# steineggerlab/unicore

Hardware: AMD Instinct MI355X
Metric: 3Di alignments/sec (cluster path) (higher is better)
Workload: dtype u16

## Files before the change

unicore_amd/csrc/uc_align.hip:

```cpp
#include <mutex>
#include <hip/hip_runtime.h>

#include <cmath>

#include <algorithm>
#include <cstdlib>
#include <cstring>

#include <rocprim/rocprim.hpp>

#include "uc_engine.h"

namespace uc {

constexpr int SW_PK_OVF_HOST = 0x7C00 - 256;

struct TbBudget {
    unsigned long long forced = 0;
    TbBudget() {
        if (const char *e = getenv("UC_TB_BUDGET_MB")) forced = std::max<unsigned long long>(1, strtoull(e, nullptr, 10)) << 20;
    }
    uint32_t segment_pairs() const { return forced ? 1000u : (32u << 20); }
    unsigned long long batch_bytes(unsigned long long total, size_t held) const {
        if (forced) return forced;
        size_t free_b = 0, total_b = 0;
        unsigned long long cap = 64ull << 30;
        if (hipMemGetInfo(&free_b, &total_b) == hipSuccess)
            cap = std::min<unsigned long long>(cap, (unsigned long long)((free_b + held) * 0.55));
        const unsigned long long budget = std::max<unsigned long long>(cap, 256ull << 20);
        if (held >= ((size_t)8 << 30)) return (unsigned long long)held - 64;
        const unsigned long long want = std::max<unsigned long long>(16ull << 30, total / 3);
        return std::min(budget, std::max<unsigned long long>(want, (unsigned long long)held));
    }
};

namespace {

constexpr int MAXCLS = 28;
struct ClassTable {
    int n;
    int cap[MAXCLS], G[MAXCLS], R[MAXCLS], pk[MAXCLS];
    uint32_t tcap[MAXCLS];
};
const ClassTable h_tab[4] = {
    {16,
     {64, 128, 192, 256, 320, 384, 448, 512, 640, 768, 896, 1024, 1280, 1536, 1792, 2048},
     {16, 16, 16, 16, 16, 16, 16, 16, 32, 32, 32, 32, 64, 64, 64, 64},
     {4, 8, 12, 16, 20, 24, 28, 32, 20, 24, 28, 32, 20, 24, 28, 32},
     {0, 0, 0, 0, 0, 0, 0, 0, 0, 0, 0, 0, 0, 0, 0, 0},
     {256, 256, 256, 256, 256, 256, 256, 256, 64, 64, 64, 64, 24, 24, 24, 24}},
    {28,
     {32, 64, 96, 128, 160, 192, 224, 256, 288, 320, 352, 384, 448, 512, 576, 640, 704, 768, 896, 1024, 1152, 1280, 1408, 1536, 1664, 1792, 1920, 2048},
     {16, 16, 16, 16, 16, 16, 16, 16, 16, 16, 16, 16, 32, 32, 32, 32, 32, 32, 64, 64, 64, 64, 64, 64, 64, 64, 64, 64},
     {2, 4, 6, 8, 10, 12, 14, 16, 18, 20, 22, 24, 14, 16, 18, 20, 22, 24, 14, 16, 18, 20, 22, 24, 26, 28, 30, 32},
     {1, 1, 1, 1, 1, 1, 1, 1, 1, 1, 1, 1, 1, 1, 1, 1, 1, 1, 1, 1, 1, 1, 1, 1, 1, 1, 1, 1},
     {64, 64, 64, 64, 64, 64, 64, 64, 64, 64, 64, 64, 64, 64, 64, 64, 64, 64, 48, 48, 48, 48, 48, 48, 24, 24, 24, 24}},
    {12,
     {64, 128, 192, 256, 384, 512, 768, 1024, 1280, 1536, 1792, 2048},
     {16, 16, 16, 16, 32, 32, 64, 64, 64, 64, 64, 64},
     {4, 8, 12, 16, 12, 16, 12, 16, 20, 24, 28, 32},
     {0, 0, 0, 0, 0, 0, 0, 0, 0, 0, 0, 0},
     {256, 256, 256, 256, 64, 64, 24, 24, 24, 24, 24, 24}},
    {16,
     {128, 256, 384, 512, 640, 768, 896, 1024, 1152, 1280, 1408, 1536, 1664, 1792, 1920, 2048},
     {64, 64, 64, 64, 64, 64, 64, 64, 64, 64, 64, 64, 64, 64, 64, 64},
     {2, 4, 6, 8, 10, 12, 14, 16, 18, 20, 22, 24, 26, 28, 30, 32},
     {1, 1, 1, 1, 1, 1, 1, 1, 1, 1, 1, 1, 1, 1, 1, 1},
     {8, 8, 8, 8, 8, 8, 16, 16, 16, 16, 16, 16, 16, 16, 16, 16}},
};
__device__ __constant__ ClassTable c_tab[4];
static int pk_known_tab(uint32_t n_pairs, uint32_t n_queries) {
    static const bool on = !(getenv("UC_SW_SPARSE") && atoi(getenv("UC_SW_SPARSE")) == 0);
    return on && (double)n_pairs < 2.5 * (double)n_queries ? 3 : 1;
}

__device__ __forceinline__ int class_of(int lq, int tab) {
    int c = 0;
    while (c < c_tab[tab].n && c_tab[tab].cap[c] < lq) c++;
    return c;
}
__device__ __forceinline__ uint32_t task_cap(int c, int tab) { return c < c_tab[tab].n ? c_tab[tab].tcap[c] : SW_LONG_TASK_PAIRS; }

__global__ void __launch_bounds__(256) plan_key_kernel(uint32_t n, const uint32_t *q, const uint32_t *t, const int32_t *qe,
                                                       const int32_t *te, const int32_t *qs, const int32_t *ts,
                                                       const uint32_t *len, int tab, uint64_t *key, uint32_t *idx,
                                                       unsigned long long *alg_bytes ) {
    unsigned long long bytes = 0, cells = 0;
    for (uint32_t i = blockIdx.x * 256 + threadIdx.x; i < n; i += gridDim.x * 256) {
        const uint32_t qq = q[i];
        const uint32_t lq = len[qq];
        const uint32_t tl = te ? (uint32_t)(te[i] + 1 - (ts ? ts[i] : 0)) : len[t[i]];
        const uint32_t ql = qe ? (uint32_t)(qe[i] + 1 - (qs ? qs[i] : 0)) : lq;
        key[i] = ((uint64_t)class_of((int)lq, tab) << 40) | ((uint64_t)qq << 16) | (uint64_t)(65535u - tl);
        idx[i] = i;
        bytes += 2ull * (ql + tl) + 32;
        cells += (unsigned long long)ql * tl;
    }
    for (int o = 32; o > 0; o >>= 1) { bytes += __shfl_down(bytes, o, 64); cells += __shfl_down(cells, o, 64); }
    if ((threadIdx.x & 63) == 0 && bytes) { atomicAdd(alg_bytes, bytes); atomicAdd(alg_bytes + 1, cells); }
}

__global__ void __launch_bounds__(256) plan_gather_kernel(uint32_t n, const uint64_t *key, const uint32_t *idx, const uint32_t *t,
                                                          const int32_t *qe, const int32_t *te, const int32_t *qs, const int32_t *ts,
                                                          uint32_t *sq, uint32_t *st, int32_t *sqe, int32_t *ste, int32_t *sqs,
                                                          int32_t *sts, uint32_t *head) {
    for (uint32_t i = blockIdx.x * 256 + threadIdx.x; i < n; i += gridDim.x * 256) {
        const uint64_t k = key[i];
        const uint32_t o = idx[i];
        sq[i] = (uint32_t)(k >> 16) & 0xFFFFFFu;
        st[i] = t[o];
        if (qe) { sqe[i] = qe[o]; ste[i] = te[o]; }
        if (qs) { sqs[i] = qs[o]; sts[i] = ts[o]; }
        head[i] = (i == 0 || (key[i - 1] >> 16) != (k >> 16)) ? i : 0u;
    }
}

__global__ void __launch_bounds__(256) plan_aux_kernel(uint32_t n, const uint32_t *idx, const int32_t *aux, int32_t *saux) {
    for (uint32_t i = blockIdx.x * 256 + threadIdx.x; i < n; i += gridDim.x * 256) saux[i] = aux[idx[i]];
}

__global__ void __launch_bounds__(256) plan_taskflag_kernel(uint32_t n, const uint64_t *key, const uint32_t *segstart, int tab, uint32_t *flag) {
    for (uint32_t i = blockIdx.x * 256 + threadIdx.x; i < n; i += gridDim.x * 256)
        flag[i] = ((i - segstart[i]) % task_cap((int)(key[i] >> 40), tab)) == 0 ? 1u : 0u;
}

__global__ void __launch_bounds__(256) plan_taskfill_kernel(uint32_t n, const uint64_t *key, const uint32_t *flag, const uint32_t *tpos,
                                                            SwTask *tasks, uint32_t *tcls) {
    for (uint32_t i = blockIdx.x * 256 + threadIdx.x; i < n; i += gridDim.x * 256) {
        if (!flag[i]) continue;
        const uint64_t k = key[i];
        const uint32_t w = tpos[i];
        tasks[w].q = (uint32_t)(k >> 16) & 0xFFFFFFu;
        tasks[w].begin = i;
        tcls[w] = (uint32_t)(k >> 40);
    }
}

__global__ void __launch_bounds__(256) plan_taskcount_kernel(uint32_t ntasks, uint32_t n, SwTask *tasks, const uint32_t *tcls,
                                                             const uint64_t *key, uint64_t *tkey, uint32_t *tidx) {
    for (uint32_t k = blockIdx.x * 256 + threadIdx.x; k < ntasks; k += gridDim.x * 256) {
        const uint32_t b = tasks[k].begin;
        const uint32_t cnt = (k + 1 < ntasks ? tasks[k + 1].begin : n) - b;
        tasks[k].count = cnt;
        const uint32_t work = cnt * (65535u - (uint32_t)(key[b] & 0xFFFF));
        tkey[k] = ((uint64_t)tcls[k] << 32) | (uint64_t)(0xFFFFFFFFu - work);
        tidx[k] = k;
    }
}

__global__ void __launch_bounds__(256) plan_taskgather_kernel(uint32_t ntasks, const uint32_t *tidx, const SwTask *in, SwTask *out) {
    for (uint32_t k = blockIdx.x * 256 + threadIdx.x; k < ntasks; k += gridDim.x * 256) out[k] = in[tidx[k]];
}

constexpr int NB = MAXCLS + 2;
__global__ void plan_bounds_kernel(uint32_t ntasks, const uint32_t *tcls, uint32_t n, const uint64_t *key, uint32_t *bounds) {
    const uint32_t c = threadIdx.x;
// ... 581 lines not shown
    UC_HIP(hipStreamSynchronize(E.stream));
    return a + b;
}

struct PackedPrefix { uint32_t pairs, tasks; };
static PackedPrefix packed_prefix(const SwPlan &P) {
    const ClassTable &tab = h_tab[P.tab];
    int c = 0;
    while (c < tab.n && tab.pk[c]) c++;
    return {P.pair_base[c], P.task_base[c]};
}

static void build_plan(Engine &E, SwPlan &P, DevBuf<char> &tmp, uint32_t n, const uint32_t *q, const uint32_t *t,
                       const int32_t *qe, const int32_t *te, int tab, const int32_t *qs = nullptr, const int32_t *ts = nullptr,
                       const int32_t *aux = nullptr ,
                       bool lpt = true ) {
    {
        static std::mutex mu;
        static bool uploaded[64] = {};
        std::lock_guard<std::mutex> g(mu);
        if (E.device < 0 || E.device >= 64 || !uploaded[E.device]) {
            ClassTable t[4];
            memcpy(t, h_tab, sizeof t);
            UC_HIP(hipMemcpyToSymbol(HIP_SYMBOL(c_tab), t, sizeof t));
            if (E.device >= 0 && E.device < 64) uploaded[E.device] = true;
        }
    }
    P.n = n; P.ntasks = 0; P.alg_bytes = 0; P.cells = 0; P.has_ends = qe != nullptr; P.has_starts = qs != nullptr; P.tab = tab;
    P.has_aux = aux != nullptr;
    memset(P.task_base, 0, sizeof P.task_base);
    memset(P.pair_base, 0, sizeof P.pair_base);
    if (!n) return;
    hipStream_t s = E.stream;
    P.key.reserve(n); P.key2.reserve(n); P.idx_in.reserve(n); P.idx.reserve(n);
    P.sq.reserve(n); P.st.reserve(n); P.head.reserve(n); P.segstart.reserve(n); P.flag.reserve(n); P.tpos.reserve(n);
    if (qe) { P.sqe.reserve(n); P.ste.reserve(n); }
    if (qs) { P.sqs.reserve(n); P.sts.reserve(n); }
    P.bytes.reserve(2); P.bounds.reserve(2 * NB);
    UC_HIP(hipMemsetAsync(P.bytes.p, 0, 16, s));
    hipLaunchKernelGGL(plan_key_kernel, grid_for(n), dim3(256), 0, s, n, q, t, qe, te, qs, ts, E.ddb.len, tab, P.key.p, P.idx_in.p, P.bytes.p);
    rocprim_call(tmp, [&](void *t, size_t &b) { return rocprim::radix_sort_pairs(t, b, P.key.p, P.key2.p, P.idx_in.p, P.idx.p, (size_t)n, 0u, 45u, s); });
    hipLaunchKernelGGL(plan_gather_kernel, grid_for(n), dim3(256), 0, s, n, P.key2.p, P.idx.p, t, qe, te, qs, ts, P.sq.p, P.st.p, P.sqe.p, P.ste.p, P.sqs.p, P.sts.p, P.head.p);
    if (aux) {
        P.saux.reserve(n);
        hipLaunchKernelGGL(plan_aux_kernel, grid_for(n), dim3(256), 0, s, n, P.idx.p, aux, P.saux.p);
    }
    max_scan_u32(E, tmp, P.head.p, P.segstart.p, n);
    hipLaunchKernelGGL(plan_taskflag_kernel, grid_for(n), dim3(256), 0, s, n, P.key2.p, P.segstart.p, tab, P.flag.p);
    P.ntasks = compact(E, tmp, P.flag.p, P.tpos.p, n);
    P.tasks.reserve(P.ntasks); P.tcls.reserve(P.ntasks);
    hipLaunchKernelGGL(plan_taskfill_kernel, grid_for(n), dim3(256), 0, s, n, P.key2.p, P.flag.p, P.tpos.p, P.tasks.p, P.tcls.p);
    P.tasks_in.reserve(P.ntasks); P.tkey.reserve(P.ntasks); P.tkey2.reserve(P.ntasks); P.tidx.reserve(P.ntasks); P.tidx2.reserve(P.ntasks);
    hipLaunchKernelGGL(plan_taskcount_kernel, grid_for(P.ntasks), dim3(256), 0, s, P.ntasks, n, P.tasks.p, P.tcls.p, P.key2.p, P.tkey.p, P.tidx.p);
    if (lpt) {
        rocprim_call(tmp, [&](void *t, size_t &b) { return rocprim::radix_sort_pairs(t, b, P.tkey.p, P.tkey2.p, P.tidx.p, P.tidx2.p, (size_t)P.ntasks, 0u, 37u, s); });
        UC_HIP(hipMemcpyAsync(P.tasks_in.p, P.tasks.p, (size_t)P.ntasks * sizeof(SwTask), hipMemcpyDeviceToDevice, s));
        hipLaunchKernelGGL(plan_taskgather_kernel, grid_for(P.ntasks), dim3(256), 0, s, P.ntasks, P.tidx2.p, P.tasks_in.p, P.tasks.p);
    }
    hipLaunchKernelGGL(plan_bounds_kernel, dim3(1), dim3(64), 0, s, P.ntasks, P.tcls.p, n, P.key2.p, P.bounds.p);
    uint32_t hb[2 * NB];
    unsigned long long bytes[2] = {0, 0};
    UC_HIP(hipMemcpyAsync(hb, P.bounds.p, sizeof hb, hipMemcpyDeviceToHost, s));
    UC_HIP(hipMemcpyAsync(bytes, P.bytes.p, 16, hipMemcpyDeviceToHost, s));
    UC_HIP(hipStreamSynchronize(s));
    UC_HIP(hipGetLastError());
    memcpy(P.task_base, hb, NB * 4);
    memcpy(P.pair_base, hb + NB, NB * 4);
    P.alg_bytes = bytes[0];
    P.cells = bytes[1];
}

static uint64_t launch_plan(Engine &E, SwPlan &P, int mode, int32_t *os, int32_t *oqe, int32_t *ote, DevBuf<int32_t> &work,
                            const uint32_t *tb = nullptr, bool only_long = false, uint32_t t0 = 0, uint32_t t1 = 0xFFFFFFFFu, bool skip_long = false) {
    const ClassTable &tab = h_tab[P.tab];
    SwArgs a;
    a.db = E.ddb; a.tasks = P.tasks.p; a.pt = P.st.p; a.pqe = P.sqe.p; a.pte = P.ste.p;
    a.pqs = P.has_starts ? P.sqs.p : nullptr; a.pts = P.has_starts ? P.sts.p : nullptr;
    a.oscore = os; a.oqe = oqe; a.ote = ote; a.open = E.p.gap_open; a.ext = E.p.gap_ext;
    if (tb) { a.tb_diag = tb[0]; a.tb_ident = tb[1]; a.tb_open = tb[2]; a.tb_ext = tb[3]; }
    a.pscore = P.has_aux ? P.saux.p : nullptr;
    const int imode = mode >= 4 ? mode - 4 : mode;
    if ((mode == 4 || mode == 6) && !P.has_aux) fail(UC_ERR_GENERIC, "known-score pass without scores");
    a.tbm = P.tbm; a.tboff = P.tboff; a.tb_band = P.tb_band;
    uint64_t launches = 0;
    const uint32_t gb = P.pair_base[tab.n], ngen = P.n - gb;
    uint32_t long_stride = 0;
    if (ngen) work.reserve(sw_long_work_ints(imode, ngen, E.max_len, &long_stride));
    UC_HIP(hipEventRecord(E.ev_fork, E.stream));
    for (int i = 0; i < E.n_streams - 1; i++) UC_HIP(hipStreamWaitEvent(E.aux[i], E.ev_fork, 0));
    int slot = 0;
    if (ngen && !skip_long) {
        SwArgs al = a;
        al.tasks = P.tasks.p + P.task_base[tab.n];
        launch_sw_long(imode, al, P.task_base[tab.n + 1] - P.task_base[tab.n], gb, work.p, long_stride, E.stream);
        UC_HIP(hipGetLastError());
        slot++;
        launches++;
    }
    for (int c = tab.n - 1; c >= 0 && !only_long; c--) {
        const uint32_t c0 = std::max(P.task_base[c], t0), c1 = std::min(P.task_base[c + 1], t1);
        if (c0 >= c1) continue;
        const uint32_t nt = c1 - c0;
        SwArgs ac = a;
        ac.tasks = P.tasks.p + c0;
        hipStream_t st = slot % E.n_streams == 0 ? E.stream : E.aux[slot % E.n_streams - 1];
        slot++;
        if (tab.pk[c]) launch_sw_pk_class(tab.G[c], tab.R[c], mode, ac, nt, st);
        else launch_sw_class(tab.G[c], tab.R[c], imode, ac, nt, st);
        UC_HIP(hipGetLastError());
        launches++;
    }
    for (int i = 0; i < E.n_streams - 1; i++) {
        UC_HIP(hipEventRecord(E.ev_join[i], E.aux[i]));
        UC_HIP(hipStreamWaitEvent(E.stream, E.ev_join[i], 0));
    }
    return launches;
}

__global__ void __launch_bounds__(256) pk_flag_kernel(uint32_t n_pk, const int32_t *os, const int32_t *oqe, int ovf, int ovf_only, uint32_t *flag) {
    for (uint32_t i = blockIdx.x * 256 + threadIdx.x; i < n_pk; i += gridDim.x * 256)
        flag[i] = (os[i] >= ovf || (!ovf_only && oqe && oqe[i] == -2)) ? 1u : 0u;
}
__global__ void __launch_bounds__(256) amb_flag_kernel(uint32_t n2, const int32_t *qe2, uint32_t *flag) {
    for (uint32_t i = blockIdx.x * 256 + threadIdx.x; i < n2; i += gridDim.x * 256) flag[i] = qe2[i] == -2 ? 1u : 0u;
}
__global__ void __launch_bounds__(256) amb_gather_kernel(uint32_t n2, const uint32_t *flag, const uint32_t *pos, const uint32_t *q2,
                                                         const uint32_t *t2, const uint32_t *link, const int32_t *s0, uint32_t *q3,
                                                         uint32_t *t3, uint32_t *link3, int32_t *s3) {
    for (uint32_t i = blockIdx.x * 256 + threadIdx.x; i < n2; i += gridDim.x * 256) {
        if (!flag[i]) continue;
        const uint32_t w = pos[i];
        q3[w] = q2[i]; t3[w] = t2[i]; link3[w] = i; s3[w] = s0[link[i]];
    }
}
__global__ void __launch_bounds__(256) amb_putback_kernel(uint32_t n3, const uint32_t *idx3, const uint32_t *link3, const uint32_t *link,
                                                          const int32_t *qe3, const int32_t *te3, int32_t *qe2, int32_t *te2,
                                                          int32_t *qe0, int32_t *te0) {
    for (uint32_t i = blockIdx.x * 256 + threadIdx.x; i < n3; i += gridDim.x * 256) {
        const uint32_t j = link3[idx3[i]];
        qe2[j] = qe3[i]; te2[j] = te3[i];
        qe0[link[j]] = qe3[i]; te0[link[j]] = te3[i];
    }
}
__global__ void __launch_bounds__(256) pk_gather_kernel(uint32_t n_pk, const uint32_t *flag, const uint32_t *pos, const uint32_t *sq,
                                                        const uint32_t *st, const int32_t *sqe, const int32_t *ste, uint32_t *q2,
                                                        uint32_t *t2, int32_t *qe2, int32_t *te2, uint32_t *link) {
    for (uint32_t i = blockIdx.x * 256 + threadIdx.x; i < n_pk; i += gridDim.x * 256) {
        if (!flag[i]) continue;
        const uint32_t w = pos[i];
        q2[w] = sq[i]; t2[w] = st[i]; link[w] = i;
        if (sqe) { qe2[w] = sqe[i]; te2[w] = ste[i]; }
    }
}
__global__ void __launch_bounds__(256) pk_putback_kernel(uint32_t n2, const uint32_t *idx2, const uint32_t *link, const int32_t *s,
                                                         const int32_t *qe, const int32_t *te, int32_t *os, int32_t *oqe, int32_t *ote) {
    for (uint32_t i = blockIdx.x * 256 + threadIdx.x; i < n2; i += gridDim.x * 256) {
        const uint32_t o = link[idx2[i]];
        os[o] = s[i];
        if (oqe) { oqe[o] = qe[i]; ote[o] = te[i]; }
    }
}


struct RerunBufs {
    DevBuf<uint32_t> flag, pos, q2, t2, link;
    DevBuf<int32_t> qe2, te2, s, qe, te, sin;
// ... 1095 lines not shown
```

unicore_amd/csrc/uc_device.h:

```cpp
#pragma once
#include <hip/hip_runtime.h>

#include <atomic>
#include <cstdint>

namespace uc {

struct PerDeviceOnce {
    std::atomic<uint64_t> mask{0};
    template <typename F>
    void operator()(F &&f) {
        int d = 0;
        (void)hipGetDevice(&d);
        const uint64_t bit = 1ull << (d & 63);
        if (!(mask.load(std::memory_order_acquire) & bit)) { f(); mask.fetch_or(bit, std::memory_order_release); }
    }
};

struct DeviceDb {
    uint32_t n = 0;
    const uint8_t *s3 = nullptr, *sa = nullptr;
    const uint16_t *lt = nullptr;
    const uint32_t *off = nullptr;
    const uint32_t *len = nullptr;
    const int8_t *S3 = nullptr, *SA = nullptr;
    const int8_t *bias = nullptr;
};

struct SwTask { uint32_t q, begin, count; };

constexpr int SW_TE_UNIQUE = 1 << 30;

struct SwArgs {
    DeviceDb db;
    const SwTask *tasks;
    const uint32_t *pt;
    const int32_t *pqe, *pte;
    const int32_t *pqs = nullptr, *pts = nullptr;
    uint8_t *tbm = nullptr;
    const unsigned long long *tboff = nullptr;
    int tb_band = 0;
    const int32_t *pscore = nullptr;
    int32_t *oscore, *oqe, *ote;
    int open, ext;
    uint32_t tb_diag = 0x10000u, tb_ident = 1u, tb_open = 0x10000u, tb_ext = 0x10000u;
};

constexpr int SW_MAX_ROWS = 2048;

struct TbBand { int nl, dlo, dhi; };
__host__ __device__ inline TbBand tb_band_of(int qs, int qe, int tl, int G, int R, int W) {
    TbBand b;
    const int d0 = qs, d1 = qe - (tl - 1);
    b.dlo = (d0 < d1 ? d0 : d1) - W;
    b.dhi = (d0 < d1 ? d1 : d0) + W;
    const int nl = (b.dhi - b.dlo + R - 1) / (R + 1) + 1;
    b.nl = (W <= 0 || nl >= G) ? G : nl;
    return b;
}

void launch_sw_class(int G, int R, int mode, const SwArgs &a, uint32_t n_tasks, hipStream_t s);
void launch_sw_pk_class(int G, int R, int mode, const SwArgs &a, uint32_t n_tasks, hipStream_t s);
constexpr uint32_t SW_LONG_TASK_PAIRS = 8;
size_t sw_long_work_ints(int mode, uint32_t n_pairs, uint32_t max_len, uint32_t *stride);
void launch_sw_long(int mode, const SwArgs &a, uint32_t n_tasks, uint32_t pair_base, int32_t *work, uint32_t stride, hipStream_t s);
void launch_ungapped(const DeviceDb &db, uint64_t n, const uint32_t *q, const uint32_t *t, const int32_t *diag,
                     int32_t *score, unsigned long long *overlap_sum , hipStream_t s);
void launch_comp_bias(const DeviceDb &db, int scale_milli, int8_t *out, hipStream_t s);
void launch_db_pad(uint32_t n, const uint32_t *off, const uint32_t *len, const uint32_t *cur ,
                   const uint64_t *roff, const uint8_t *r3, const uint8_t *ra,
                   uint64_t total, uint8_t *s3, uint8_t *sa, uint16_t *lt, hipStream_t s);

}
```

unicore_amd/csrc/uc_sw_pk_impl.hpp:

```cpp
#pragma once
#include <hip/hip_runtime.h>

#include "uc_device.h"
#include "uc_sw_impl.hpp"

namespace uc {

constexpr int SW_PK_OVF = 0x7C00 - 256;

typedef uint16_t u16x2_t __attribute__((ext_vector_type(2)));
typedef uint32_t u32x4_u __attribute__((ext_vector_type(4), aligned(4)));
typedef uint32_t u32x2_u __attribute__((ext_vector_type(2), aligned(4)));
typedef const uint32_t __attribute__((address_space(4))) *sw_cu32p;
__device__ __forceinline__ u16x2_t pk_v(uint32_t x) { return __builtin_bit_cast(u16x2_t, x); }
__device__ __forceinline__ uint32_t pk_u(u16x2_t v) { return __builtin_bit_cast(uint32_t, v); }
__device__ __forceinline__ uint32_t pk_add_sat(uint32_t a, uint32_t b) { return pk_u(__builtin_elementwise_add_sat(pk_v(a), pk_v(b))); }
__device__ __forceinline__ uint32_t pk_sub_sat(uint32_t a, uint32_t b) { return pk_u(__builtin_elementwise_sub_sat(pk_v(a), pk_v(b))); }
__device__ __forceinline__ uint32_t pk_max(uint32_t a, uint32_t b) { return pk_u(__builtin_elementwise_max(pk_v(a), pk_v(b))); }
__device__ __forceinline__ uint32_t pk_min(uint32_t a, uint32_t b) {
    uint32_t r;
    asm("v_pk_min_u16 %0, %1, %2" : "=v"(r) : "v"(a), "v"(b));
    return r;
}
__device__ __forceinline__ uint32_t pk_max3(uint32_t a, uint32_t b, uint32_t c) {
    uint32_t r;
    asm("v_pk_maximum3_f16 %0, %1, %2, %3" : "=v"(r) : "v"(a), "v"(b), "v"(c));
    return r;
}

template <int G, int R, int MODE, int NW>
__global__ void __launch_bounds__(NW * 64) sw_pk_kernel(const SwArgs a) {
    constexpr bool TBB = MODE == 7;
    constexpr bool KNOWN = MODE == 4 || MODE == 6;
    constexpr int BASE = KNOWN ? MODE - 4 : (TBB ? 0 : MODE);
    constexpr bool TRACK = BASE != 1 && !TBB, MASK = BASE == 2 || TBB, REVQ = BASE != 0, REVT = BASE == 2;
    constexpr int RW = (R + 3) / 4, BW = RW | 1, RSW = G * BW, NT = NW * 64;
    static_assert(R % 2 == 0 && R <= 32, "R must be even, <= 32");
    extern __shared__ __attribute__((aligned(16))) uint32_t lds[];
    uint32_t *P3 = lds, *PA = lds + SW_NLET * RSW;
    uint32_t *slot_ctr = lds + 2 * SW_NLET * RSW;

    const SwTask task = a.tasks[blockIdx.x];
    const int tid = threadIdx.x, lane = tid & 63;
    const int g = lane % G;
    const uint32_t qoff = a.db.off[task.q];
    const int lq = (int)a.db.len[task.q];
    const uint32_t open2 = (uint32_t)a.open * 0x10001u, ext2 = (uint32_t)a.ext * 0x10001u, bias2 = 128u * 0x10001u;
    const uint32_t nslots = (task.count + 1) >> 1;

    for (int idx = tid; idx < SW_NLET * G * RW; idx += NT) {
        const int c = idx / (G * RW), rem = idx % (G * RW), gg = rem / RW, k = rem % RW;
        uint32_t w3 = 0, wa = 0;
#pragma unroll
        for (int b = 0; b < 4; b++) {
            const int row = gg * R + 4 * k + b;
            if (row < lq && c < 21 && 4 * k + b < R) {
                const int qi = REVQ ? lq - 1 - row : row;
                const int q3 = a.db.s3[qoff + qi], qa = a.db.sa[qoff + qi];
                w3 |= (uint32_t)(a.db.S3[q3 * 21 + c] + 64) << (8 * b);
                wa |= (uint32_t)(a.db.SA[qa * 21 + c] + 64) << (8 * b);
            }
        }
        P3[c * RSW + gg * BW + k] = w3;
        PA[c * RSW + gg * BW + k] = wa;
    }
    if (tid == 0) *slot_ctr = 0;
    __syncthreads();

    uint32_t H[R], E[R], rowbest[(TRACK && !KNOWN) ? R : 1];
    uint32_t mskA[MASK ? RW : 1], mskB[MASK ? RW : 1];
    uint32_t best = 0, Hlast = 0, prevHup = 0, fout = 0;
    int colA = -1, colB = -1;
    [[maybe_unused]] int rowA = 0, rowB = 0;
    [[maybe_unused]] bool multA = false, multB = false;
    [[maybe_unused]] uint32_t knownA = 0, knownB = 0;
    uint32_t gA = 0, gB = 0, toffA = 0, toffB = 0;
    [[maybe_unused]] unsigned long long tbA = 0, tbB = 0;
    [[maybe_unused]] int tsaA = 0, tsbA = 0, tsaB = 0, tsbB = 0;
    [[maybe_unused]] uint32_t trowA = 0, trowB = 0, tslotA = 0, tslotB = 0;
    int tlenA = 0, tlenB = 0, rowoffA = 0, rowoffB = 0;
    bool vB = false, active = false;
    int lst = 0, nst = 0;
    uint32_t c1 = 0, cin = 0;
    struct RawLetters { uint32_t a3, aa, b3, ba; } r2 = {0, 0, 0, 0};
    uint32_t nA3[RW], nAa[RW], nB3[RW], nBa[RW];
    [[maybe_unused]] const uint16_t *ltA = nullptr, *ltB = nullptr;

    auto issue_letters = [&](int st) -> RawLetters {
        RawLetters r;
        if constexpr (G == 64) {
            const int ia = max(min(st, tlenA - 1), 0), ib = max(min(st, tlenB - 1), 0);
            const uint32_t pa = toffA + (uint32_t)(REVT ? max(tlenA - 1 - ia, 0) : ia);
            const uint32_t pb_ = toffB + (uint32_t)(REVT ? max(tlenB - 1 - ib, 0) : ib);
            auto ld = [&](const uint8_t *base, uint32_t p) -> uint32_t {
                const sw_cu32p w = (sw_cu32p)(uintptr_t)(base + (p & ~3u));
                return (*w >> (8u * (p & 3u))) & 0xffu;
            };
            r.a3 = ld(a.db.s3, pa); r.aa = ld(a.db.sa, pa); r.b3 = ld(a.db.s3, pb_); r.ba = ld(a.db.sa, pb_);
        } else {
            const uint32_t ia = REVT ? (uint32_t)max(tlenA - st, 0) : (uint32_t)min(st, tlenA);
            const uint32_t ib = REVT ? (uint32_t)max(tlenB - st, 0) : (uint32_t)min(st, tlenB);
            r.a3 = ltA[ia]; r.b3 = ltB[ib];
            r.aa = 0; r.ba = 0;
        }
        return r;
    };
    auto pack_letters = [&](const RawLetters &r, int st) -> uint32_t {
        if constexpr (G == 64) {
            const uint32_t ca_ = st < tlenA ? (r.a3 | (r.aa << 8)) : SW_PADPACK;
            const uint32_t cb_ = st < tlenB ? (r.b3 | (r.ba << 8)) : SW_PADPACK;
            return ca_ | (cb_ << 16);
        } else if constexpr (TBB) {
            return (st < tlenA ? r.a3 : SW_PADPACK) | ((st < tlenB ? r.b3 : SW_PADPACK) << 16);
        } else {
            return r.a3 | (r.b3 << 16);
        }
    };
    uint32_t off3 = (uint32_t)(g * BW) * 4u, offa = (uint32_t)(SW_NLET * RSW + g * BW) * 4u;
    asm volatile("" : "+v"(off3), "+v"(offa));
    auto fetch_profile = [&]() __attribute__((always_inline)) {
        const char *l8 = (const char *)lds;
        const uint32_t *pA3 = (const uint32_t *)(l8 + (cin & 0xff) * (RSW * 4) + off3), *pAa = (const uint32_t *)(l8 + ((cin >> 8) & 0xff) * (RSW * 4) + offa);
        const uint32_t *pB3 = (const uint32_t *)(l8 + ((cin >> 16) & 0xff) * (RSW * 4) + off3), *pBa = (const uint32_t *)(l8 + (cin >> 24) * (RSW * 4) + offa);
#pragma unroll
        for (int k = 0; k < RW; k++) { nA3[k] = pA3[k]; nAa[k] = pAa[k]; nB3[k] = pB3[k]; nBa[k] = pBa[k]; }
    };

    auto start_slot = [&]() {
        uint32_t idx = 0;
        if (g == 0) idx = atomicAdd(slot_ctr, 1u);
        if constexpr (G == 64) idx = (uint32_t)__builtin_amdgcn_readfirstlane((int)idx);
        else idx = (uint32_t)__shfl((int)idx, lane - g, 64);
        active = idx < nslots;
        if (!active) return;
        const uint32_t iA = 2 * idx, iB = iA + 1;
        vB = iB < task.count;
        gA = task.begin + iA;
        gB = task.begin + (vB ? iB : iA);
        const uint32_t tA = a.pt[gA], tB = a.pt[gB];
        toffA = a.db.off[tA]; toffB = a.db.off[tB];
        tlenA = REVT ? a.pte[gA] + 1 : (int)a.db.len[tA];
        tlenB = vB ? (REVT ? a.pte[gB] + 1 : (int)a.db.len[tB]) : 0;
        if constexpr (TBB) {
            toffA += (uint32_t)a.pts[gA]; toffB += (uint32_t)a.pts[gB];
            tlenA = a.pte[gA] - a.pts[gA] + 1;
            tlenB = vB ? a.pte[gB] - a.pts[gB] + 1 : 0;
            tbA = a.tboff[gA]; tbB = a.tboff[gB];
            const int qsA = a.pqs[gA], qeA = a.pqe[gA], qsB = a.pqs[gB], qeB = a.pqe[gB];
            {
                constexpr int RBc = 4 * RW;
                const TbBand bA = tb_band_of(qsA, qeA, tlenA, G, R, a.tb_band), bB = tb_band_of(qsB, qeB, vB ? tlenB : 1, G, R, a.tb_band);
                const bool fullA = bA.nl >= G, fullB = bB.nl >= G;
                tsaA = fullA ? 0 : g * (R + 1) - bA.dhi; tsbA = fullA ? 0x7fffffff : g * (R + 1) + R - 1 - bA.dlo;
                tsaB = fullB ? 0 : g * (R + 1) - bB.dhi; tsbB = fullB ? 0x7fffffff : g * (R + 1) + R - 1 - bB.dlo;
                trowA = (uint32_t)(bA.nl * RBc); trowB = (uint32_t)(bB.nl * RBc);
                tslotA = (uint32_t)((g % bA.nl) * RBc); tslotB = (uint32_t)((g % bB.nl) * RBc);
            }
#pragma unroll
            for (int k = 0; k < RW; k++) {
                uint32_t ma = 0, mb = 0;
#pragma unroll
                for (int b = 0; b < 4; b++) {
                    const int row = g * R + 4 * k + b;
                    ma |= (row >= qsA && row <= qeA ? 0xFFu : 0u) << (8 * b);
                    mb |= (row >= qsB && row <= qeB ? 0xFFu : 0u) << (8 * b);
                }
                mskA[k] = ma; mskB[k] = mb;
            }
        } else if constexpr (MASK) {
            rowoffA = lq - 1 - a.pqe[gA];
            rowoffB = lq - 1 - a.pqe[gB];
#pragma unroll
            for (int k = 0; k < RW; k++) {
                uint32_t ma = 0, mb = 0;
#pragma unroll
                for (int b = 0; b < 4; b++) {
                    ma |= (g * R + 4 * k + b >= rowoffA ? 0xFFu : 0u) << (8 * b);
                    mb |= (g * R + 4 * k + b >= rowoffB ? 0xFFu : 0u) << (8 * b);
                }
                mskA[k] = ma; mskB[k] = mb;
            }
        }
        if constexpr (G != 64) {
            ltA = a.db.lt + toffA - (REVT ? 1 : 0);
            ltB = vB ? a.db.lt + toffB - (REVT ? 1 : 0) : a.db.lt + toffA - 1;
        }
#pragma unroll
        for (int r = 0; r < R; r++) { H[r] = 0; E[r] = 0; }
        if constexpr (TRACK && !KNOWN) {
#pragma unroll
            for (int r = 0; r < R; r++) rowbest[r] = 0;
        }
        if constexpr (KNOWN) {
            knownA = (uint32_t)a.pscore[gA];
            knownB = vB ? (uint32_t)a.pscore[gB] : 0u;
            rowA = 0; rowB = 0; multA = false; multB = false;
        }
        best = 0; colA = -1; colB = -1; Hlast = 0; prevHup = 0; fout = 0;
        lst = 0;
        nst = (max(tlenA, tlenB) + G) & ~1;
        c1 = pack_letters(issue_letters(1), 1);
        r2 = issue_letters(2);
        if constexpr (G == 64) {
            c1 = (uint32_t)__builtin_amdgcn_readfirstlane((int)c1);
            r2.a3 = (uint32_t)__builtin_amdgcn_readfirstlane((int)r2.a3); r2.aa = (uint32_t)__builtin_amdgcn_readfirstlane((int)r2.aa);
            r2.b3 = (uint32_t)__builtin_amdgcn_readfirstlane((int)r2.b3); r2.ba = (uint32_t)__builtin_amdgcn_readfirstlane((int)r2.ba);
        }
        cin = (uint32_t)shift_from_prev_lane<G>((int)(SW_PADPACK * 0x10001u), (int)pack_letters(issue_letters(0), 0), g);
        fetch_profile();
    };

    auto do_step = [&](const int st, const bool ODD) __attribute__((always_inline)) {
        uint32_t sA[RW], sB[RW];
#pragma unroll
        for (int k = 0; k < RW; k++) {
            sA[k] = nA3[k] + nAa[k];
            sB[k] = nB3[k] + nBa[k];
            if constexpr (MASK) { sA[k] &= mskA[k]; sB[k] &= mskB[k]; }
        }
        cin = (uint32_t)shift_from_prev_lane<G>((int)cin, (int)c1, g);
        c1 = pack_letters(r2, st + 2);
        r2 = issue_letters(st + 3);
        fetch_profile();
        const uint32_t Hup = (uint32_t)shift_from_prev_lane_zero<G>((int)Hlast, g);
        uint32_t f = (uint32_t)shift_from_prev_lane_zero<G>((int)fout, g);
        uint32_t diag = prevHup;
        uint32_t colmax = 0;
        [[maybe_unused]] uint32_t code[TBB ? R : 1];
#pragma unroll
        for (int r = 0; r < R; r++) {
            const uint32_t ub = __builtin_amdgcn_perm(sB[r >> 2], sA[r >> 2], 0x0c000c00u | ((4u + (r & 3)) << 16) | (uint32_t)(r & 3));
            const uint32_t x = pk_sub_sat(pk_add_sat(diag, ub), bias2);
            const uint32_t e = E[r];
            const uint32_t h = pk_max3(x, e, f);
            const uint32_t hprev = H[r];
            diag = hprev;
            H[r] = h;
            const uint32_t t = pk_sub_sat(h, open2);
            const uint32_t esub = pk_sub_sat(e, ext2), fsub = pk_sub_sat(f, ext2);
            if constexpr (TBB) code[r] = h;
            E[r] = pk_max(esub, t);
            f = pk_max(fsub, t);
            if constexpr (TRACK && !KNOWN) { if (ODD) rowbest[r] = pk_max3(rowbest[r], hprev, h); }
            if (r & 1) colmax = pk_max3(colmax, H[r - 1], h);
        }
        if constexpr (TBB) {
            uint32_t wa[RW], wb[RW];
#pragma unroll
            for (int k = 0; k < RW; k++) {
                const uint32_t c0 = code[4 * k], c1_ = 4 * k + 1 < R ? code[4 * k + 1] : 0u;
                const uint32_t c2 = 4 * k + 2 < R ? code[4 * k + 2] : 0u, c3 = 4 * k + 3 < R ? code[4 * k + 3] : 0u;
                const uint32_t p01 = __builtin_amdgcn_perm(c1_, c0, 0x06020400u);
                const uint32_t p23 = __builtin_amdgcn_perm(c3, c2, 0x06020400u);
                wa[k] = __builtin_amdgcn_perm(p23, p01, 0x05040100u);
// ... 48 lines not shown
        Hlast = H[R - 1];
        fout = f;
        prevHup = Hup;
    };

    auto finish_slot = [&]() {
        if constexpr (TBB) return;
        if constexpr (KNOWN) {
#pragma unroll
            for (int half = 0; half < 2; half++) {
                const int col = half ? colB : colA, row = half ? rowB : rowA;
                int key = col < 0 ? 0x7fffffff : ((col << 11) | (g * R + row));
                int nrows = (col < 0 ? 0 : 1) + ((half ? multB : multA) ? G : 0);
#pragma unroll
                for (int m = 1; m < G; m <<= 1) {
                    key = min(key, __shfl_xor(key, m, 64));
                    nrows += __shfl_xor(nrows, m, 64);
                }
                const bool valid = half ? vB : true;
                const uint32_t gp = half ? gB : gA;
                if (g == 0 && valid) {
                    const int rowoff = half ? rowoffB : rowoffA;
                    const bool found = key != 0x7fffffff;
                    a.oscore[gp] = (int)(half ? knownB : knownA);
                    a.oqe[gp] = found ? (key & 2047) - rowoff : -2;
                    a.ote[gp] = found ? ((key >> 11) | ((MODE == 6 && nrows == 1) ? SW_TE_UNIQUE : 0)) : -2;
                }
            }
            return;
        }
#pragma unroll
        for (int half = 0; half < 2; half++) {
            int score = half ? (int)(best >> 16) : (int)(best & 0xffffu);
            int col = half ? colB : colA;
#pragma unroll
            for (int m = 1; m < G; m <<= 1) {
                const int os = __shfl_xor(score, m, 64), oc = __shfl_xor(col, m, 64);
                const bool take = os > score || (os == score && oc < col);
                score = take ? os : score;
                col = take ? oc : col;
            }
            int cnt = 0, minrow = 1 << 30;
            if constexpr (TRACK) {
#pragma unroll
                for (int r = R - 1; r >= 0; r--) {
                    const int rb = half ? (int)(rowbest[r] >> 16) : (int)(rowbest[r] & 0xffffu);
                    if (rb == score) { cnt++; minrow = g * R + r; }
                }
#pragma unroll
                for (int m = 1; m < G; m <<= 1) {
                    cnt += __shfl_xor(cnt, m, 64);
                    minrow = min(minrow, __shfl_xor(minrow, m, 64));
                }
            }
            const bool valid = half ? vB : true;
            const uint32_t gp = half ? gB : gA;
            if (g == 0 && valid) {
                a.oscore[gp] = score;
                if constexpr (TRACK) {
                    const int rowoff = half ? rowoffB : rowoffA;
                    int qe = -1, te = -1;
                    if (score > 0) { te = col; qe = (cnt == 1 && score < SW_PK_OVF) ? minrow - rowoff : -2; }
                    a.oqe[gp] = qe;
                    a.ote[gp] = te;
                }
            }
        }
    };

    start_slot();
    while (__builtin_amdgcn_ballot_w64(active) != 0) {
        if (active) {
            do_step(lst, false);
            do_step(lst + 1, true);
            lst += 2;
            if (lst >= nst) {
                finish_slot();
                start_slot();
            }
        }
    }
}

template <int MODE>
void launch_sw_pk_class_mode(int G, int R, const SwArgs &a, uint32_t n_tasks, hipStream_t s) {
#define UC_SW_CASE(GG, RR)                                                                              \
    if (G == GG && R == RR) {                                                                           \
        constexpr int BW = (((RR + 3) / 4) | 1);                                                        \
         \
        constexpr int NW = GG == 16 ? 2 : (GG == 32 ? 4 : (RR < 14 ? 2 : 8));                           \
        const size_t lds = (size_t)2 * SW_NLET * GG * BW * 4 + 16;                                      \
        static PerDeviceOnce once;                                                                      \
        if (lds > 64 * 1024)                                                                            \
            once([&] { (void)hipFuncSetAttribute((const void *)sw_pk_kernel<GG, RR, MODE, NW>,           \
                                                 hipFuncAttributeMaxDynamicSharedMemorySize, (int)lds); }); \
        hipLaunchKernelGGL((sw_pk_kernel<GG, RR, MODE, NW>), dim3(n_tasks), dim3(NW * 64), lds, s, a);  \
        return;                                                                                         \
    }
    UC_SW_CASE(16, 2) UC_SW_CASE(16, 4) UC_SW_CASE(16, 6) UC_SW_CASE(16, 8) UC_SW_CASE(16, 10) UC_SW_CASE(16, 12)
    UC_SW_CASE(16, 14) UC_SW_CASE(16, 16) UC_SW_CASE(16, 18) UC_SW_CASE(16, 20) UC_SW_CASE(16, 22) UC_SW_CASE(16, 24)
    UC_SW_CASE(32, 14) UC_SW_CASE(32, 16) UC_SW_CASE(32, 18) UC_SW_CASE(32, 20) UC_SW_CASE(32, 22) UC_SW_CASE(32, 24)
    UC_SW_CASE(64, 14) UC_SW_CASE(64, 16) UC_SW_CASE(64, 18) UC_SW_CASE(64, 20) UC_SW_CASE(64, 22) UC_SW_CASE(64, 24)
    UC_SW_CASE(64, 26) UC_SW_CASE(64, 28) UC_SW_CASE(64, 30) UC_SW_CASE(64, 32)
    if constexpr (MODE == 4 || MODE == 6) {
        UC_SW_CASE(64, 2) UC_SW_CASE(64, 4) UC_SW_CASE(64, 6) UC_SW_CASE(64, 8) UC_SW_CASE(64, 10) UC_SW_CASE(64, 12)
    }
#undef UC_SW_CASE
    fprintf(stderr, "unicore-cluster: no packed SW kernel for class (G=%d, R=%d)\n", G, R);
    abort();
}

template <int MODE>
void preload_sw_pk_mode() {
    hipFuncAttributes fa;
    (void)hipFuncGetAttributes(&fa, (const void *)sw_pk_kernel<64, 14, MODE, 8>);
}

}
```

Before: 21.65 million.

## Pack two query tasks per workgroup in sparse known-score SW kernel

Adds a two-query variant of the packed Smith-Waterman kernel for the sparse known-score table with G=64. Each workgroup builds two query profiles in LDS and spreads the pairs of two consecutive tasks across its wave slots. This targets workgroups that sit mostly idle when a query has only one or two pairs, and it halves the grid size. In exchange it doubles LDS per workgroup, which can reduce occupancy, and adds per-slot selection logic.

```diff
diff --git a/unicore_amd/csrc/uc_align.hip b/unicore_amd/csrc/uc_align.hip
--- a/unicore_amd/csrc/uc_align.hip
+++ b/unicore_amd/csrc/uc_align.hip
@@ -69,9 +69,17 @@
      {8, 8, 8, 8, 8, 8, 16, 16, 16, 16, 16, 16, 16, 16, 16, 16}},
 };
 __device__ __constant__ ClassTable c_tab[4];
+static bool sw_sparse_on() {
+    const char *e = getenv("UC_SW_SPARSE");
+    return !(e && atoi(e) == 0);
+}
 static int pk_known_tab(uint32_t n_pairs, uint32_t n_queries) {
-    static const bool on = !(getenv("UC_SW_SPARSE") && atoi(getenv("UC_SW_SPARSE")) == 0);
-    return on && (double)n_pairs < 2.5 * (double)n_queries ? 3 : 1;
+    return sw_sparse_on() && (double)n_pairs < 2.5 * (double)n_queries ? 3 : 1;
+}
+static bool sw_two_query(int tab, int mode) {
+    if (tab != 3 || (mode != 4 && mode != 6) || !sw_sparse_on()) return false;
+    const char *e = getenv("UC_SW_TWO_QUERY");
+    return !(e && atoi(e) == 0);
 }
 
 __device__ __forceinline__ int class_of(int lq, int tab) {
@@ -819,6 +827,7 @@
     const int imode = mode >= 4 ? mode - 4 : mode;
     if ((mode == 4 || mode == 6) && !P.has_aux) fail(UC_ERR_GENERIC, "known-score pass without scores");
     a.tbm = P.tbm; a.tboff = P.tboff; a.tb_band = P.tb_band;
+    a.pair_tasks = sw_two_query(P.tab, mode) ? 1u : 0u;
     uint64_t launches = 0;
     const uint32_t gb = P.pair_base[tab.n], ngen = P.n - gb;
     uint32_t long_stride = 0;
diff --git a/unicore_amd/csrc/uc_device.h b/unicore_amd/csrc/uc_device.h
--- a/unicore_amd/csrc/uc_device.h
+++ b/unicore_amd/csrc/uc_device.h
@@ -44,6 +44,7 @@
     int32_t *oscore, *oqe, *ote;
     int open, ext;
     uint32_t tb_diag = 0x10000u, tb_ident = 1u, tb_open = 0x10000u, tb_ext = 0x10000u;
+    uint32_t pair_tasks = 0;
 };
 
 constexpr int SW_MAX_ROWS = 2048;
diff --git a/unicore_amd/csrc/uc_sw_pk_impl.hpp b/unicore_amd/csrc/uc_sw_pk_impl.hpp
--- a/unicore_amd/csrc/uc_sw_pk_impl.hpp
+++ b/unicore_amd/csrc/uc_sw_pk_impl.hpp
@@ -28,41 +28,57 @@
     return r;
 }
 
-template <int G, int R, int MODE, int NW>
+template <int G, int R, int MODE, int NW, bool TQ = false>
 __global__ void __launch_bounds__(NW * 64) sw_pk_kernel(const SwArgs a) {
     constexpr bool TBB = MODE == 7;
     constexpr bool KNOWN = MODE == 4 || MODE == 6;
     constexpr int BASE = KNOWN ? MODE - 4 : (TBB ? 0 : MODE);
     constexpr bool TRACK = BASE != 1 && !TBB, MASK = BASE == 2 || TBB, REVQ = BASE != 0, REVT = BASE == 2;
     constexpr int RW = (R + 3) / 4, BW = RW | 1, RSW = G * BW, NT = NW * 64;
+    constexpr int PROF = 2 * SW_NLET * RSW;
     static_assert(R % 2 == 0 && R <= 32, "R must be even, <= 32");
+    static_assert(!TQ || KNOWN, "two-query workgroups exist for the known-score modes only");
     extern __shared__ __attribute__((aligned(16))) uint32_t lds[];
     uint32_t *P3 = lds, *PA = lds + SW_NLET * RSW;
-    uint32_t *slot_ctr = lds + 2 * SW_NLET * RSW;
-
-    const SwTask task = a.tasks[blockIdx.x];
+    uint32_t *slot_ctr = lds + (TQ ? 2 : 1) * PROF;
+
+    const SwTask task = a.tasks[TQ ? 2 * blockIdx.x : blockIdx.x];
+    [[maybe_unused]] SwTask task2 = {task.q, task.begin, 0};
+    if constexpr (TQ) {
+        if (2 * blockIdx.x + 1 < a.pair_tasks) task2 = a.tasks[2 * blockIdx.x + 1];
+    }
     const int tid = threadIdx.x, lane = tid & 63;
     const int g = lane % G;
     const uint32_t qoff = a.db.off[task.q];
     const int lq = (int)a.db.len[task.q];
+    [[maybe_unused]] const uint32_t qoff2 = TQ ? a.db.off[task2.q] : 0u;
+    [[maybe_unused]] const int lq2 = TQ ? (int)a.db.len[task2.q] : 0;
+    const uint32_t npairs = TQ ? task.count + task2.count : task.count;
     const uint32_t open2 = (uint32_t)a.open * 0x10001u, ext2 = (uint32_t)a.ext * 0x10001u, bias2 = 128u * 0x10001u;
-    const uint32_t nslots = (task.count + 1) >> 1;
-
-    for (int idx = tid; idx < SW_NLET * G * RW; idx += NT) {
+    const uint32_t nslots = (npairs + 1) >> 1;
+
+    constexpr int NPROF = SW_NLET * G * RW;
+    const int nbuild = TQ && task2.count ? 2 * NPROF : NPROF;
+    for (int idx0 = tid; idx0 < nbuild; idx0 += NT) {
+        int idx = idx0, pl = lq;
+        uint32_t po = qoff, *p3 = P3, *pa = PA;
+        if constexpr (TQ) {
+            if (idx0 >= NPROF) { idx -= NPROF; pl = lq2; po = qoff2; p3 += PROF; pa += PROF; }
+        }
         const int c = idx / (G * RW), rem = idx % (G * RW), gg = rem / RW, k = rem % RW;
         uint32_t w3 = 0, wa = 0;
 #pragma unroll
         for (int b = 0; b < 4; b++) {
             const int row = gg * R + 4 * k + b;
-            if (row < lq && c < 21 && 4 * k + b < R) {
-                const int qi = REVQ ? lq - 1 - row : row;
-                const int q3 = a.db.s3[qoff + qi], qa = a.db.sa[qoff + qi];
+            if (row < pl && c < 21 && 4 * k + b < R) {
+                const int qi = REVQ ? pl - 1 - row : row;
+                const int q3 = a.db.s3[po + qi], qa = a.db.sa[po + qi];
                 w3 |= (uint32_t)(a.db.S3[q3 * 21 + c] + 64) << (8 * b);
                 wa |= (uint32_t)(a.db.SA[qa * 21 + c] + 64) << (8 * b);
             }
         }
-        P3[c * RSW + gg * BW + k] = w3;
-        PA[c * RSW + gg * BW + k] = wa;
+        p3[c * RSW + gg * BW + k] = w3;
+        pa[c * RSW + gg * BW + k] = wa;
     }
     if (tid == 0) *slot_ctr = 0;
     __syncthreads();
@@ -118,10 +134,13 @@
     };
     uint32_t off3 = (uint32_t)(g * BW) * 4u, offa = (uint32_t)(SW_NLET * RSW + g * BW) * 4u;
     asm volatile("" : "+v"(off3), "+v"(offa));
+    [[maybe_unused]] uint32_t off3A = off3, offaA = offa, off3B = off3, offaB = offa;
+    [[maybe_unused]] int lqA = lq, lqB = lq;
     auto fetch_profile = [&]() __attribute__((always_inline)) {
         const char *l8 = (const char *)lds;
-        const uint32_t *pA3 = (const uint32_t *)(l8 + (cin & 0xff) * (RSW * 4) + off3), *pAa = (const uint32_t *)(l8 + ((cin >> 8) & 0xff) * (RSW * 4) + offa);
-        const uint32_t *pB3 = (const uint32_t *)(l8 + ((cin >> 16) & 0xff) * (RSW * 4) + off3), *pBa = (const uint32_t *)(l8 + (cin >> 24) * (RSW * 4) + offa);
+        const uint32_t o3A = TQ ? off3A : off3, oaA = TQ ? offaA : offa, o3B = TQ ? off3B : off3, oaB = TQ ? offaB : offa;
+        const uint32_t *pA3 = (const uint32_t *)(l8 + (cin & 0xff) * (RSW * 4) + o3A), *pAa = (const uint32_t *)(l8 + ((cin >> 8) & 0xff) * (RSW * 4) + oaA);
+        const uint32_t *pB3 = (const uint32_t *)(l8 + ((cin >> 16) & 0xff) * (RSW * 4) + o3B), *pBa = (const uint32_t *)(l8 + (cin >> 24) * (RSW * 4) + oaB);
 #pragma unroll
         for (int k = 0; k < RW; k++) { nA3[k] = pA3[k]; nAa[k] = pAa[k]; nB3[k] = pB3[k]; nBa[k] = pBa[k]; }
     };
@@ -134,9 +153,19 @@
         active = idx < nslots;
         if (!active) return;
         const uint32_t iA = 2 * idx, iB = iA + 1;
-        vB = iB < task.count;
-        gA = task.begin + iA;
-        gB = task.begin + (vB ? iB : iA);
+        vB = iB < npairs;
+        if constexpr (TQ) {
+            const uint32_t jB = vB ? iB : iA;
+            const bool sA = iA >= task.count, sB = jB >= task.count;
+            gA = sA ? task2.begin + (iA - task.count) : task.begin + iA;
+            gB = sB ? task2.begin + (jB - task.count) : task.begin + jB;
+            lqA = sA ? lq2 : lq; lqB = sB ? lq2 : lq;
+            off3A = off3 + (sA ? PROF * 4u : 0u); offaA = offa + (sA ? PROF * 4u : 0u);
+            off3B = off3 + (sB ? PROF * 4u : 0u); offaB = offa + (sB ? PROF * 4u : 0u);
+        } else {
+            gA = task.begin + iA;
+            gB = task.begin + (vB ? iB : iA);
+        }
         const uint32_t tA = a.pt[gA], tB = a.pt[gB];
         toffA = a.db.off[tA]; toffB = a.db.off[tB];
         tlenA = REVT ? a.pte[gA] + 1 : (int)a.db.len[tA];
@@ -168,8 +197,8 @@
                 mskA[k] = ma; mskB[k] = mb;
             }
         } else if constexpr (MASK) {
-            rowoffA = lq - 1 - a.pqe[gA];
-            rowoffB = lq - 1 - a.pqe[gB];
+            rowoffA = (TQ ? lqA : lq) - 1 - a.pqe[gA];
+            rowoffB = (TQ ? lqB : lq) - 1 - a.pqe[gB];
 #pragma unroll
             for (int k = 0; k < RW; k++) {
                 uint32_t ma = 0, mb = 0;
@@ -384,6 +413,8 @@
     }
 }
 
+constexpr size_t SW_PK_LDS_MAX = 160 * 1024;
+
 template <int MODE>
 void launch_sw_pk_class_mode(int G, int R, const SwArgs &a, uint32_t n_tasks, hipStream_t s) {
 #define UC_SW_CASE(GG, RR)                                                                              \
@@ -391,11 +422,24 @@
         constexpr int BW = (((RR + 3) / 4) | 1);                                                        \
          \
         constexpr int NW = GG == 16 ? 2 : (GG == 32 ? 4 : (RR < 14 ? 2 : 8));                           \
-        const size_t lds = (size_t)2 * SW_NLET * GG * BW * 4 + 16;                                      \
+        constexpr size_t lds = (size_t)2 * SW_NLET * GG * BW * 4 + 16;                                  \
         static PerDeviceOnce once;                                                                      \
         if (lds > 64 * 1024)                                                                            \
             once([&] { (void)hipFuncSetAttribute((const void *)sw_pk_kernel<GG, RR, MODE, NW>,           \
                                                  hipFuncAttributeMaxDynamicSharedMemorySize, (int)lds); }); \
+        if constexpr ((MODE == 4 || MODE == 6) && GG == 64 && 2 * (lds - 16) + 16 <= SW_PK_LDS_MAX) {   \
+            if (a.pair_tasks) {                                                                         \
+                constexpr size_t lds2 = 2 * (lds - 16) + 16;                                            \
+                static PerDeviceOnce once2;                                                             \
+                if (lds2 > 64 * 1024)                                                                   \
+                    once2([&] { (void)hipFuncSetAttribute((const void *)sw_pk_kernel<GG, RR, MODE, NW, true>, \
+                                                          hipFuncAttributeMaxDynamicSharedMemorySize, (int)lds2); }); \
+                SwArgs a2 = a;                                                                          \
+                a2.pair_tasks = n_tasks;                                                                \
+                hipLaunchKernelGGL((sw_pk_kernel<GG, RR, MODE, NW, true>), dim3((n_tasks + 1) / 2), dim3(NW * 64), lds2, s, a2); \
+                return;                                                                                 \
+            }                                                                                           \
+        }                                                                                               \
         hipLaunchKernelGGL((sw_pk_kernel<GG, RR, MODE, NW>), dim3(n_tasks), dim3(NW * 64), lds, s, a);  \
         return;                                                                                         \
     }
```

Measured after the change: 21.25 million. 0.982x the previous value.
